# smpurkis/PyTorch-Face-Detection-from-Scratch

Hardware: AMD Instinct MI355X
Metric: train imgs/sec (PoolResnet 480^2, bs=256 per GPU) (higher is better)
Workload: dtype f32 (3x3 convs: bf16x3 split MFMA, fp32 accumulate)

## Files before the change

### pytorch-face-detection-from-scratch_amd/csrc/fdet_conv3x3_ps.hip

```cpp
#include "fdet_conv3x3_x3.h"
#include "fdet_ps.h"
#include "fdet_ldsdma.h"
#include <algorithm>

using namespace fdet;

typedef __attribute__((address_space(3))) void* lds_void_t;
typedef const __attribute__((address_space(1))) void* glb_void_t;
typedef unsigned u32x4 __attribute__((ext_vector_type(4)));

namespace {

#ifndef PS_DBG
#define PS_DBG 0
#endif
constexpr int PSA = 9 * 2 * 64;
constexpr int PS_ROWI = 10;

enum { PSE_FWD_FULL = 0, PSE_DGRAD_ACT = 1, PSE_FWD_POOL = 2, PSE_DGRAD_ADDPOOL = 3 };

struct PsConvArgs {
  const bf16x8* x;
  const bf16x8* a_hi;
  const bf16x8* a_lo;
// ... 5 lines not shown
  float* pool_f32;
  unsigned char* route_out;
  const float* dout;
  const unsigned char* route_in;
  float* dx_f32;
  int Hp, Wp, HPp, WPp, plane_p, img_p;
  int Nimg, last0, Wlast, Wf, Wpf, xo;
  unsigned magic_nimg;
  int N, H, W, HP;
  int nch, ntiles;
  int plane_i, img_i, plane_o, img_o;
  unsigned magic_hp;
  float slope;
};

typedef unsigned u32x2_t __attribute__((ext_vector_type(2)));

__device__ __forceinline__ void ps_keep(const f32x16& v) {
#if defined(__HIP_DEVICE_COMPILE__)
  asm volatile("" ::"v"(v));
#endif
}

__device__ __forceinline__ void ps_acc_read(const f32x16& acc, const int r, float& z) {
#if defined(__HIP_DEVICE_COMPILE__)
  asm("v_accvgpr_read_b32 %0, %1" : "=v"(z) : "a"(acc[r]));
#else
  z = acc[r];
#endif
}

template <int MODE, bool P16>
__device__ __forceinline__ void ps_unit(const f32x16& acc, const int gp, const float (&bza)[4], const float (&bzb)[4],
                                        const u32x2_t (&sg)[2], const float slope, const bool ok, const int ob, const int m,
                                        const int half, const int gstride, const int plane_o_bytes,
                                        const __amdgpu_buffer_rsrc_t yrs) {
  float za[4], zb[4];
#pragma unroll
  for (int i = 0; i < 4; ++i) {
#if defined(__HIP_DEVICE_COMPILE__)
    asm("v_accvgpr_read_b32 %0, %1" : "=v"(za[i]) : "a"(acc[8 * gp + i]));
    asm("v_accvgpr_read_b32 %0, %1" : "=v"(zb[i]) : "a"(acc[8 * gp + 4 + i]));
#else
    za[i] = acc[8 * gp + i]; zb[i] = acc[8 * gp + 4 + i];
#endif
  }
// ... 14 lines not shown
  unsigned ha[2], la[2], hb[2], lb[2];
  if (P16) {
    ps_hi4(za, ha);
    ps_hi4(zb, hb);
  } else {
    ps_split4(za, ha, la);
    ps_split4(zb, hb, lb);
  }
#pragma unroll
  for (int k = 0; k < 2; ++k) {
    auto r1 = __builtin_amdgcn_permlane32_swap(ha[k], hb[k], false, false);
    ha[k] = r1[0]; hb[k] = r1[1];
    if (!P16) {
      auto r2 = __builtin_amdgcn_permlane32_swap(la[k], lb[k], false, false);
      la[k] = r2[0]; lb[k] = r2[1];
    }
  }
  const int G = 4 * m + 2 * gp + half;
  const unsigned off = ok ? (unsigned)(ob + G * gstride) * 16u : 0x80000000u;
  __builtin_amdgcn_raw_buffer_store_b128(u32x4{ha[0], ha[1], hb[0], hb[1]}, yrs, off, 0, 0);
  if (!P16) __builtin_amdgcn_raw_buffer_store_b128(u32x4{la[0], la[1], lb[0], lb[1]}, yrs, off, plane_o_bytes, 0);
}

template <int MODE, int WP, bool P16>
__global__ void __launch_bounds__(256, 1)
k_conv3x3_ps(const PsConvArgs p) {
  constexpr bool WOVEN = MODE == PSE_FWD_FULL || MODE == PSE_DGRAD_ACT || MODE == PSE_DGRAD_ADDPOOL;
  extern __shared__ __attribute__((aligned(16))) char smem[];
  bf16x8* const lds = reinterpret_cast<bf16x8*>(smem);
  const int tid = threadIdx.x, lane = tid & 63;
  const int wid = __builtin_amdgcn_readfirstlane(tid >> 6);
  const int l31 = lane & 31, half = lane >> 5;
  constexpr int WPL = WP == 64 ? 6 : 5, R = 512 / WP, PT = (R + 2) * WP + 8, NBI = (R + 2) * WP / 64;
  constexpr int buf_units = 2 * PSA + 4 * PT;
  const int HP = p.HP;
  int qn[4];
#pragma unroll
  for (int n = 0; n < 4; ++n) qn[n] = WP == 64 ? (2 * wid + (n & 1)) * 64 + (n >> 1) * 32 : (4 * wid + n) * 32;
  constexpr bool POOLM = MODE == PSE_FWD_POOL || MODE == PSE_DGRAD_ADDPOOL;
  if (POOLM) {
#pragma unroll
    for (int n = 0; n < 4; ++n) qn[n] = (WP == 64 ? (2 * wid + (n >> 1)) * 64 : (4 * wid + (n >> 1)) * 32) + (n & 1);
  }
  const int lb = POOLM ? (WP == 64 ? 2 * l31 : 2 * l31 + 32 * (l31 >> 4)) : l31;
  int tile = blockIdx.x, tend = p.ntiles, tstep = gridDim.x;
  if ((gridDim.x & 7) == 0) {
    const int grp = blockIdx.x & 7, chunk = (p.ntiles + 7) >> 3;
    tile = grp * chunk + (blockIdx.x >> 3);
    tend = min((grp + 1) * chunk, p.ntiles);
// ... 24 lines not shown
    _Pragma("unroll") for (int k_ = 0; k_ < ((PS_DBG & 16) ? 0 : 9); ++k_)                          \
      dma_piece(ad_ + k_ * 1024, wvoff, wrs, (unsigned)(C) * (PSA * 16) + k_ * 1024);              \
    const unsigned bso_ = (unsigned)((wid >> 1) * p.plane_i + (2 * (C) + (wid & 1)) * HP * WP) * 16u; \
    const unsigned bd_ = db_ + (unsigned)(2 * PSA + wid * PT) * 16u;                               \
    _Pragma("unroll") for (int i_ = 0; i_ < NBI; ++i_) dma_piece(bd_ + i_ * 1024, ro[i_], xrs, bso_); \
  }

  f32x16 accA[2][4], accB[WOVEN ? 2 : 1][WOVEN ? 4 : 1];
  if (WOVEN) {
#pragma unroll
    for (int m = 0; m < 2; ++m)
#pragma unroll
      for (int n = 0; n < 4; ++n)
#pragma unroll
        for (int r = 0; r < 16; ++r) accB[WOVEN ? m : 0][WOVEN ? n : 0][r] = 0.f;
  }

  float bz[2][4][4];
#pragma unroll
  for (int m = 0; m < 2; ++m)
#pragma unroll
    for (int g = 0; g < 4; ++g)
#pragma unroll
      for (int i = 0; i < 4; ++i) bz[m][g][i] = (MODE == PSE_FWD_FULL || MODE == PSE_FWD_POOL) ? p.bias[32 * m + 8 * g + 4 * half + i] : 0.f;

  const int a_off = half * 64 + l31;
  const int b_off = 2 * PSA + half * PT + lb;
  const int gstride = HP * WP, plane_o_bytes = p.plane_o * 16;
  const __amdgpu_buffer_rsrc_t yrs = __builtin_amdgcn_make_buffer_rsrc(p.y, 0, (int)((size_t)p.N * p.img_o * 16), 0x00020000);

  int ob[4];
  bool okn[4];
#pragma unroll
  for (int n = 0; n < 4; ++n) { ob[n] = 0; okn[n] = false; }
#define PS_GEO(T)                                                                                  \
  {                                                                                                \
    _Pragma("unroll") for (int n_ = 0; n_ < 4; ++n_) {                                             \
      const int q_ = qn[n_] + l31;                                                                 \
      const int col_ = q_ & (WP - 1);                                                              \
      const int v_ = (T) * R + (q_ >> WPL);                                                        \
      const int nn_ = (int)__umulhi((unsigned)v_, p.magic_hp), y_ = v_ - nn_ * HP;                 \
      okn[n_] = nn_ < p.N && y_ < p.H && col_ < (nn_ >= p.last0 ? p.Wlast : p.W);                  \
      ob[n_] = nn_ * p.img_o + y_ * WP + col_ + 1;                                                 \
    }                                                                                              \
  }
  u32x2_t sgp[4][2][2][2];
#pragma unroll
// ... 16 lines not shown
  }

  int young = 0;
  int sb = 0;
#define PS_WAITN(K) else if (young == K) asm volatile("s_waitcnt vmcnt(" #K ")" ::: "memory");
#define PS_OPEN()                                                                                  \
  {                                                                                                \
    if (young == 0) asm volatile("s_waitcnt vmcnt(0)" ::: "memory");                               \
    PS_WAITN(4) PS_WAITN(8) PS_WAITN(12) PS_WAITN(16) PS_WAITN(32) PS_WAITN(36) PS_WAITN(40) PS_WAITN(44) PS_WAITN(48) PS_WAITN(63) \
    else asm volatile("s_waitcnt vmcnt(0)" ::: "memory");                                          \
    __builtin_amdgcn_s_barrier();                                                                  \
  }
#define PS_NEXT(C)                                                                                 \
  {                                                                                                \
    if ((C) + 1 < p.nch) {                                                                         \
      PS_DMA((C) + 1, sb ^ 1)                                                                      \
    } else if (tile + tstep < tend) {                                                              \
      PS_ROWOFF(tile + tstep)                                                                      \
      PS_DMA(0, sb ^ 1)                                                                            \
    }                                                                                              \
    __builtin_amdgcn_sched_barrier(0);                                                             \
  }
  bf16x8 ah[2][2], al[2][2], bh[2][4], bl[2][4];
#define PS_FRAGS(F, T)                                                                             \
  {                                                                                                \
    const int to_ = ((T) / 3) * WP + (T) % 3;                                                      \
    _Pragma("unroll") for (int m_ = 0; m_ < 2; ++m_) {                                             \
      ah[F][m_] = Aw[(T) * 128 + m_ * 32];                                                         \
      if (!P16) al[F][m_] = Aw[PSA + (T) * 128 + m_ * 32];                                         \
    }                                                                                              \
    _Pragma("unroll") for (int n_ = 0; n_ < 4; ++n_) {                                             \
      bh[F][n_] = Bw[qn[n_] + to_];                                                                \
      if (!P16) bl[F][n_] = Bw[2 * PT + qn[n_] + to_];                                             \
    }                                                                                              \
  }
#define PS_BODY(ACC, FIRST, JOB, PREV)                                                             \
  {                                                                                                \
    const bf16x8* buf_ = lds + sb * buf_units;                                                     \
    const bf16x8* Aw = buf_ + a_off;                                                               \
    const bf16x8* Bw = buf_ + b_off;                                                               \
    PS_FRAGS(0, 0)                                                                                 \
    __builtin_amdgcn_sched_barrier(0);                                                             \
    _Pragma("unroll") for (int t = 0; t < 9; ++t) {                                                \
      const int F = t & 1;                                                                         \
      if (t < 8) PS_FRAGS(F ^ 1, t + 1)                                                            \
      if (!(PS_DBG & 2)) {                                                                         \
        _Pragma("unroll") for (int m = 0; m < 2; ++m)                                              \
// ... 41 lines not shown
          if (i < 6) __builtin_amdgcn_sched_group_barrier(0x100, 1, 0);                            \
          if ((JOB) != 0) __builtin_amdgcn_sched_group_barrier(0x002, 6, 0);                       \
          if ((JOB) != 0 && (i >= 7 || (MODE == PSE_DGRAD_ADDPOOL && i >= 4))) __builtin_amdgcn_sched_group_barrier(0x040, 1, 0); \
        }                                                                                          \
      } else {                                                                                     \
      _Pragma("unroll") for (int i = 0; i < 12; ++i) {                                             \
        __builtin_amdgcn_sched_group_barrier(0x008, 1, 0);                                         \
        __builtin_amdgcn_sched_group_barrier(0x100, 1, 0);                                         \
        if ((JOB) != 0) __builtin_amdgcn_sched_group_barrier(0x002, 3, 0);                         \
      }                                                                                            \
      _Pragma("unroll") for (int i = 0; i < 12; ++i) {                                             \
        __builtin_amdgcn_sched_group_barrier(0x008, 1, 0);                                         \
        if ((JOB) != 0) __builtin_amdgcn_sched_group_barrier(0x002, 3, 0);                         \
        if ((JOB) != 0 && (i >= 10 || (MODE == PSE_DGRAD_ADDPOOL && i >= 8))) __builtin_amdgcn_sched_group_barrier(0x040, 1, 0); \
      }                                                                                            \
      }                                                                                            \
    }                                                                                              \
    sb ^= 1;                                                                                       \
  }
  const __amdgpu_buffer_rsrc_t prs = __builtin_amdgcn_make_buffer_rsrc(MODE == PSE_FWD_POOL ? (void*)p.pool_ps : (void*)p.dx_f32, 0,
      MODE == PSE_FWD_POOL ? (int)((size_t)p.N * p.img_p * 16) : (int)((size_t)p.Nimg * 64 * p.H * p.Wf * 4), 0x00020000);
  const __amdgpu_buffer_rsrc_t frs = __builtin_amdgcn_make_buffer_rsrc(p.pool_f32, 0, (int)((size_t)p.Nimg * 64 * p.Hp * p.Wpf * 4), 0x00020000);
  const __amdgpu_buffer_rsrc_t rrs = __builtin_amdgcn_make_buffer_rsrc(p.route_out, 0, (int)((size_t)p.N * 64 * p.Hp * p.Wp), 0x00020000);
  const int pool_cnt = MODE == PSE_FWD_POOL ? 4 * ((P16 ? 1 : 2) * (p.pool_ps != nullptr) + (p.route_out != nullptr) + 8 * (p.pool_f32 != nullptr)) : 63;
#define PS_WIN(T)                                                                                  \
    const int rb_ = WP == 64 ? 2 * wid : 4 * wid + 2 * (l31 >> 4);                                 \
    const int v_ = (T) * R + rb_;                                                                  \
    const int nn = (int)__umulhi((unsigned)v_, p.magic_hp), y = v_ - nn * HP;                      \
    const int xp = WP == 64 ? l31 : (l31 & 15), yp = y >> 1;                                       \
    const bool okw = nn < p.N && y < p.H && 2 * xp < (nn >= p.last0 ? p.Wlast : p.W);              \
                \
    const int si = p.last0 == 0 ? 0 : (p.Nimg == 1 ? nn : (int)__umulhi((unsigned)nn, p.magic_nimg)); \
    const int ni = nn - si * p.Nimg, xg = si * (p.xo >> 1) + xp;
  float dgp[2][2][2][4];
  unsigned rkp[2][2][2];
  unsigned sto = 0x80000000u;
#pragma unroll
  for (int m = 0; m < 2; ++m)
#pragma unroll
    for (int gp = 0; gp < 2; ++gp)
#pragma unroll
      for (int ab = 0; ab < 2; ++ab) {
        rkp[m][gp][ab] = 0u;
#pragma unroll
        for (int i = 0; i < 4; ++i) dgp[m][gp][ab][i] = 0.f;
      }
#define PS_POOLPREF(T)                                                                             \
  {                                                                                                \
    PS_WIN(T)                                                                                      \
    const int HWp = p.Hp * p.Wpf, HWr = p.Hp * p.Wp;                                               \
    const int pbase = okw ? (ni * 64 * p.Hp + yp) * p.Wpf + xg : 0;                                \
    const int rbase = okw ? (nn * 8 * p.Hp + yp) * p.Wp + xp : 0;                                  \
    _Pragma("unroll") for (int m = 0; m < 2; ++m)                                                  \
      _Pragma("unroll") for (int gp = 0; gp < 2; ++gp)                                             \
        _Pragma("unroll") for (int ab = 0; ab < 2; ++ab) {                                         \
          const int G = 4 * m + 2 * gp + ab;                                                       \
          _Pragma("unroll") for (int i = 0; i < 4; ++i) {                                          \
            const float v_ = p.dout[pbase + (8 * G + 4 * half + i) * HWp];                         \
            dgp[m][gp][ab][i] = okw ? v_ : 0.f;                                                    \
          }                                                                                        \
          rkp[m][gp][ab] = *reinterpret_cast<const unsigned*>(p.route_in + (size_t)(rbase + G * HWr) * 8 + 4 * half); \
        }                                                                                          \
    sto = okw ? (unsigned)(((ni * 64 + 4 * half) * p.H + y) * p.Wf + 2 * xg) * 4u : 0x80000000u;   \
  }
#define PS_EPI_FWD_POOL(ACC, T)                                                                    \
  if (!(PS_DBG & 1)) {                                                                             \
    PS_WIN(T)                                                                                      \
    const int sb0 = okw ? nn * p.img_i + y * WP + 2 * xp + 1 : 0;                                  \
    u32x2_t sk[2][2][4][4];                                                                        \
    float scv[2][2][2][4];                                                                         \
    _Pragma("unroll") for (int m = 0; m < 2; ++m)                                                  \
      _Pragma("unroll") for (int gp = 0; gp < 2; ++gp) {                                           \
        const size_t ga = (size_t)(4 * m + 2 * gp) * gstride, gb = ga + (size_t)gstride;           \
        _Pragma("unroll") for (int n = 0; n < 4; ++n) {                                            \
          const u32x2_t* ap = reinterpret_cast<const u32x2_t*>(p.aux + sb0 + (n >> 1) * WP + (n & 1)) + half; \
          sk[m][gp][n][0] = ap[ga * 2];                                                            \
          sk[m][gp][n][1] = P16 ? u32x2_t{0u, 0u} : ap[(ga + p.plane_i) * 2];                      \
          sk[m][gp][n][2] = ap[gb * 2];                                                            \
          sk[m][gp][n][3] = P16 ? u32x2_t{0u, 0u} : ap[(gb + p.plane_i) * 2];                      \
        }                                                                                          \
        _Pragma("unroll") for (int i = 0; i < 4; ++i) {                                            \
          const int ch = 32 * m + 16 * gp + 4 * half + i;                                          \
          scv[m][gp][0][i] = (p.scale && okw) ? p.scale[ni * 64 + ch] : 1.f;                       \
          scv[m][gp][1][i] = (p.scale && okw) ? p.scale[ni * 64 + ch + 8] : 1.f;                   \
        }                                                                                          \
      }                                                                                            \
     \
     \
    float pvs[2][2][2][4];                                                                         \
    unsigned rts[2][2][2];                                                                         \
    _Pragma("unroll") for (int m = 0; m < 2; ++m)                                                  \
      _Pragma("unroll") for (int gp = 0; gp < 2; ++gp) {                                           \
        unsigned rt[2] = {0u, 0u};                                                                 \
        _Pragma("unroll") for (int ab = 0; ab < 2; ++ab)                                           \
          _Pragma("unroll") for (int i = 0; i < 4; ++i) {                                          \
            float mx = -INFINITY;                                                                  \
            int arg = 0;                                                                           \
            unsigned bits = 0;                                                                     \
            _Pragma("unroll") for (int n = 0; n < 4; ++n) {                                        \
              float z;                                                                             \
              ps_acc_read(ACC[m][n], 8 * gp + 4 * ab + i, z);                                      \
              const float w_ = z + bz[m][2 * gp + ab][i];                                          \
              z = fmaxf(w_, w_ * p.slope);                                                         \
              bits |= (z > 0.f ? 1u : 0u) << n;                                                    \
              const float u_ = z * scv[m][gp][ab][i] + ps_join(sk[m][gp][n][2 * ab][i >> 1], sk[m][gp][n][2 * ab + 1][i >> 1], i & 1); \
              if (u_ > mx || u_ != u_) { mx = u_; arg = n; }    \
            }                                                                                      \
            pvs[m][gp][ab][i] = mx;                                                                \
            rt[ab] |= (bits | ((unsigned)arg << 4)) << (8 * i);                                    \
          }                                                                                        \
        rts[m][gp][0] = rt[0]; rts[m][gp][1] = rt[1];                                              \
      }                                                                                            \
    if (p.pool_f32) {                 \
      _Pragma("unroll") for (int m = 0; m < 2; ++m)                                                \
        _Pragma("unroll") for (int gp = 0; gp < 2; ++gp) {                                         \
          const unsigned off = okw ? (unsigned)(((ni * 64 + 32 * m + 16 * gp + 4 * half) * p.Hp + yp) * p.Wpf + xg) * 4u : 0x80000000u; \
          _Pragma("unroll") for (int jj = 0; jj < 8; ++jj)                                         \
            __builtin_amdgcn_raw_buffer_store_b32(__builtin_bit_cast(unsigned, pvs[m][gp][jj >> 2][jj & 3]), frs, off, \
                                                  (8 * (jj >> 2) + (jj & 3)) * p.Hp * p.Wpf * 4, 0); \
        }                                                                                          \
    }                                                                                              \
     \
    _Pragma("unroll") for (int m = 0; m < 2; ++m)                                                  \
      _Pragma("unroll") for (int gp = 0; gp < 2; ++gp) {                                           \
        _Pragma("unroll") for (int i = 0; i < 4; ++i) {                                            \
          auto r_ = __builtin_amdgcn_permlane32_swap(__float_as_uint(pvs[m][gp][0][i]), __float_as_uint(pvs[m][gp][1][i]), false, false); \
          const unsigned r0_ = r_[0], r1_ = r_[1];    \
          pvs[m][gp][0][i] = __uint_as_float(r0_); pvs[m][gp][1][i] = __uint_as_float(r1_);        \
        }                                                                                          \
        { auto r_ = __builtin_amdgcn_permlane32_swap(rts[m][gp][0], rts[m][gp][1], false, false); rts[m][gp][0] = r_[0]; rts[m][gp][1] = r_[1]; } \
      }                                                                                            \
    if (p.pool_ps) {                                                                               \
      _Pragma("unroll") for (int m = 0; m < 2; ++m)                                                \
        _Pragma("unroll") for (int gp = 0; gp < 2; ++gp) {                                         \
          const int G = 4 * m + 2 * gp + half;                                                     \
          unsigned ha[2], la[2], hb[2], lb2[2];                                                    \
          if (P16) { ps_hi4(pvs[m][gp][0], ha); ps_hi4(pvs[m][gp][1], hb); }                       \
          else { ps_split4(pvs[m][gp][0], ha, la); ps_split4(pvs[m][gp][1], hb, lb2); }            \
          const unsigned off = okw ? (unsigned)(nn * p.img_p + (G * p.HPp + yp) * p.WPp + xp + 1) * 16u : 0x80000000u; \
          __builtin_amdgcn_raw_buffer_store_b128(u32x4{ha[0], ha[1], hb[0], hb[1]}, prs, off, 0, 0); \
          if (!P16) __builtin_amdgcn_raw_buffer_store_b128(u32x4{la[0], la[1], lb2[0], lb2[1]}, prs, off, p.plane_p * 16, 0); \
        }                                                                                          \
    }                                                                                              \
    if (p.route_out) {                                                                             \
      _Pragma("unroll") for (int m = 0; m < 2; ++m)                                                \
        _Pragma("unroll") for (int gp = 0; gp < 2; ++gp) {                                         \
          const int G = 4 * m + 2 * gp + half;                                                     \
          const unsigned off = okw ? (unsigned)(((nn * 8 + G) * p.Hp + yp) * p.Wp + xp) * 8u : 0x80000000u; \
          __builtin_amdgcn_raw_buffer_store_b64(u32x2_t{rts[m][gp][0], rts[m][gp][1]}, rrs, off, 0, 0); \
        }                                                                                          \
    }                                                                                              \
  } else {                                                                                         \
    _Pragma("unroll") for (int m = 0; m < 2; ++m)                                                  \
      _Pragma("unroll") for (int n = 0; n < 4; ++n) ps_keep(ACC[m][n]);                            \
  }
#define PS_EPI_ADDPOOL(ACC, T)                                                                     \
  if (!(PS_DBG & 1)) {                                                                             \
    PS_WIN(T)                                                                                      \
    float dg[2][2][2][4];                                                                          \
    unsigned rk[2][2][2];                                                                          \
    const int HWp = p.Hp * p.Wpf;                                                                  \
    const int pbase = okw ? (ni * 64 * p.Hp + yp) * p.Wpf + xg : 0;                                \
    _Pragma("unroll") for (int m = 0; m < 2; ++m)                                                  \
      _Pragma("unroll") for (int gp = 0; gp < 2; ++gp)                                             \
        _Pragma("unroll") for (int ab = 0; ab < 2; ++ab) {                                         \
          const int G = 4 * m + 2 * gp + ab;                                                       \
          _Pragma("unroll") for (int i = 0; i < 4; ++i) dg[m][gp][ab][i] = okw ? p.dout[pbase + (8 * G + 4 * half + i) * HWp] : 0.f; \
          rk[m][gp][ab] = okw ? *reinterpret_cast<const unsigned*>(p.route_in + (size_t)(((nn * 8 + G) * p.Hp + yp) * p.Wp + xp) * 8 + 4 * half) : 0u; \
        }                                                                                          \
    _Pragma("unroll") for (int m = 0; m < 2; ++m)                                                  \
      _Pragma("unroll") for (int gp = 0; gp < 2; ++gp)                                             \
        _Pragma("unroll") for (int ab = 0; ab < 2; ++ab)                                           \
          _Pragma("unroll") for (int i = 0; i < 4; ++i) {                                          \
// ... 41 lines not shown
      PS_OPEN()                                                                                    \
      PS_NEXT(c)                                                                                   \
      PS_BODY(ACC, 0, 0, PREV)                                                                     \
      young = 0;                                                                                   \
    }                                                                                              \
    PS_GEO(tile)                                                                                   \
    etile = tile;                                                                                  \
    if (WOVEN && MODE == PSE_DGRAD_ACT && !(PS_DBG & 1)) {                                         \
      PS_SIGNS()                                                                                   \
      young += 32;                                                                                 \
    }                                                                                              \
    if constexpr (MODE == PSE_DGRAD_ADDPOOL) {                                                     \
      if (!(PS_DBG & 1)) {                                                                         \
        PS_POOLPREF(tile)                                                                          \
        young = min(young + 40, 63);                                                               \
      }                                                                                            \
    }                                                                                              \
    if (!WOVEN) {                                                                                  \
      PS_EPILOGUE(ACC)                                                                             \
      young = (PS_DBG & 1) ? 0 : (POOLM ? pool_cnt : 32);                                          \
    }                                                                                              \
  }

  int etile = tile;
  PS_ROWOFF(tile)
  PS_DMA(0, 0)
  if (WOVEN) {
    for (;;) {
      PS_TILE(accA, accB)
      tile += tstep;
      if (tile >= tend) { PS_EPILOGUE(accA) break; }
      PS_TILE(accB, accA)
      tile += tstep;
      if (tile >= tend) { PS_EPILOGUE(accB) break; }
    }
  } else {
    for (; tile < tend; tile += tstep) PS_TILE(accA, accA)
  }
#undef PS_TILE
#undef PS_EPILOGUE
#undef PS_EPI_ADDPOOL
#undef PS_EPI_FWD_POOL
#undef PS_POOLPREF
#undef PS_WIN
#undef PS_WAITN
#undef PS_BODY
#undef PS_FRAGS
#undef PS_NEXT
#undef PS_OPEN
#undef PS_GEO
#undef PS_SIGNS
#undef PS_DMA
#undef PS_ROWOFF
}

#ifndef PS_TU
#define PS_TU (-1)
#endif
#define PS_CAT_(a, b) a##b
#define PS_CAT(a, b) PS_CAT_(a, b)
#define PS_TU_NAME PS_CAT(fdet_ps_launch_, PS_TU)
template <int MODE, int WP, bool P16>
int launch_ps(const PsConvArgs& p, size_t lds, int grid, hipStream_t st) {
  static bool attr_set = false;
  constexpr int lds_max = 2 * (2 * PSA + 4 * 648) * 16;
  if (!attr_set) {
    if ((int)lds > lds_max || hipFuncSetAttribute((const void*)k_conv3x3_ps<MODE, WP, P16>, hipFuncAttributeMaxDynamicSharedMemorySize, lds_max) != hipSuccess) {
      (void)hipGetLastError();
      return fail(FDET_ELAUNCH, "conv3x3_ps: cannot reserve %zu bytes of LDS", lds);
    }
    attr_set = true;
  }
  hipLaunchKernelGGL((k_conv3x3_ps<MODE, WP, P16>), dim3(grid), dim3(256), lds, st, p);
  return check_launch("fdet_conv3x3_ps");
}

}
#define PS_DECL_LAUNCH(N) extern "C" int fdet_ps_launch_##N(const void* args, size_t lds, int grid, void* stream);
PS_DECL_LAUNCH(0) PS_DECL_LAUNCH(1) PS_DECL_LAUNCH(2) PS_DECL_LAUNCH(3) PS_DECL_LAUNCH(4) PS_DECL_LAUNCH(5) PS_DECL_LAUNCH(6) PS_DECL_LAUNCH(7)
PS_DECL_LAUNCH(8) PS_DECL_LAUNCH(9) PS_DECL_LAUNCH(10) PS_DECL_LAUNCH(11) PS_DECL_LAUNCH(12) PS_DECL_LAUNCH(13) PS_DECL_LAUNCH(14) PS_DECL_LAUNCH(15)
#if PS_TU >= 0
extern "C" int PS_TU_NAME(const void* args, size_t lds, int grid, void* stream) {
  return launch_ps<(PS_TU & 7) / 2, (PS_TU & 1) ? 64 : 32, (PS_TU >= 8)>(*reinterpret_cast<const PsConvArgs*>(args), lds, grid, (hipStream_t)stream);
}
#endif
namespace {
#if PS_TU == -1
typedef int (*ps_launch_fn)(const void*, size_t, int, void*);
const ps_launch_fn PS_LAUNCHERS[16] = {fdet_ps_launch_0, fdet_ps_launch_1, fdet_ps_launch_2, fdet_ps_launch_3,
                                       fdet_ps_launch_4, fdet_ps_launch_5, fdet_ps_launch_6, fdet_ps_launch_7,
                                       fdet_ps_launch_8, fdet_ps_launch_9, fdet_ps_launch_10, fdet_ps_launch_11,
                                       fdet_ps_launch_12, fdet_ps_launch_13, fdet_ps_launch_14, fdet_ps_launch_15};
struct PsPoolIO {
  const float* scale = nullptr; void* pool_ps = nullptr; float* pool_f32 = nullptr; unsigned char* route_out = nullptr;
  const float* dout = nullptr; const unsigned char* route_in = nullptr; float* dx_f32 = nullptr;
};

const char* ps_conv_refusal(int pooled, int N, int Cin, int Cout, int H, int W) {
  PsGeo gi, go, gp;
  PsStrips sp, spo;
  if (!(Cout == 64 && Cin % 16 == 0 && Cin >= 32)) return "Cout must be 64 and Cin a multiple of 16, at least 32";
  if (!(ps_geo_strips(N, Cin, H, W, gi, sp) && ps_geo_strips(N, Cout, H, W, go, spo) && gi.WP >= 32 && sp.Ws + 2 <= gi.WP))
    return "unsupported map (W + 2 <= 32 or 64 slots, or an even width in strips)";
  if (!((size_t)(gi.N + 2) * gi.img * 16 < ((size_t)1 << 32) && (size_t)(go.N + 2) * go.img * 16 < ((size_t)1 << 32)))
    return "tensor too large for the 32-bit byte offsets of the DMA descriptors";
  if (pooled) {
    if ((H & 1) || (W & 1) || Cin != 64) return "pooled block: even map and 64 channels required";
    if ((size_t)N * 64 * H * W * 4 >= ((size_t)1 << 31)) return "pooled block: tensor too large for 32-bit offsets";
    if (pooled == 2 && sp.S != 1) return "a strip map writes its pooled output as fp32 NCHW (pool_f32)";
    if (pooled == 2 && !ps_geo(gi.N, 64, H / 2, W / 2, gp)) return "the pooled map has no PS layout";
  }
  if ((long)gi.N * gi.HP + gi.HP >= (1 << 20)) return "too many rows";
  return nullptr;
}

// ... 18 lines not shown
  p.bias = bias;
  p.y = reinterpret_cast<bf16x8*>(y);
  p.aux = reinterpret_cast<const bf16x8*>(aux);
  p.scale = io.scale; p.pool_ps = reinterpret_cast<bf16x8*>(io.pool_ps); p.pool_f32 = io.pool_f32; p.route_out = io.route_out;
  p.dout = io.dout; p.route_in = io.route_in; p.dx_f32 = io.dx_f32;
  p.Hp = H / 2; p.Wp = W / 2; p.HPp = p.WPp = p.plane_p = p.img_p = 0;
  p.Nimg = Nimg; p.last0 = sp.S > 1 ? (sp.S - 1) * Nimg : 0; p.Wlast = sp.Wlast; p.Wf = Wfull; p.Wpf = Wfull / 2; p.xo = sp.Ws;
  p.magic_nimg = Nimg > 1 ? magic_of(Nimg) : 0u;
  PsGeo go;
  PsStrips spo;
  ps_geo_strips(Nimg, Cout, H, Wfull, go, spo);
  if (pool_mode == 2) {
    ps_geo(N, 64, H / 2, W / 2, gp);
    p.HPp = gp.HP; p.WPp = gp.WP; p.plane_p = gp.plane; p.img_p = gp.img;
  }
  p.N = N; p.H = H; p.W = W; p.HP = gi.HP;
  p.nch = Cin / 16;
  const int R = 512 / gi.WP, PT = (R + 2) * gi.WP + 8;
  const long vr = (long)N * gi.HP;
  p.ntiles = (int)((vr + R - 1) / R);
  p.plane_i = gi.plane; p.img_i = gi.img; p.plane_o = go.plane; p.img_o = go.img;
  p.magic_hp = magic_of(gi.HP);
  p.slope = slope;
  const size_t lds = (size_t)2 * (2 * PSA + 4 * PT) * 16;
  const int grid = std::min(p.ntiles, num_cus());
  const bool w64 = gi.WP == 64;
  switch (mode) {
    case PSE_FWD_FULL:
      FDET_REQUIRE(bias, "conv3x3_ps_fwd: bias is required");
      break;
    case PSE_DGRAD_ACT:
      FDET_REQUIRE(aux, "conv3x3_ps_dgrad_act: the activation is required");
      break;
    case PSE_FWD_POOL:
      FDET_REQUIRE(bias && aux && (io.pool_ps || io.pool_f32), "conv3x3_ps_fwd_pool: bias, skip and an output are required");
      break;
    default:
      FDET_REQUIRE(io.dout && io.route_in && io.dx_f32, "conv3x3_ps_dgrad_unpool: dout, route and dx are required");
      break;
  }
  return PS_LAUNCHERS[(p16 ? 8 : 0) + 2 * mode + (w64 ? 1 : 0)](&p, lds, grid, (void*)st);
}
#endif

}

#if PS_TU == -1
extern "C" int fdet_conv3x3_ps_ok(int N, int Cin, int Cout, int H, int W, int pooled) {
  return ps_conv_refusal(pooled, N, Cin, Cout, H, W) == nullptr;
}

extern "C" int fdet_conv3x3_ps_fwd(const void* x_ps, const void* wpk, const float* bias, void* y_ps, int N, int Cin,
                                   int Cout, int H, int W, float slope, void* stream) {
  return run_ps(PSE_FWD_FULL, x_ps, wpk, bias, nullptr, y_ps, PsPoolIO{}, N, Cin, Cout, H, W, slope, (hipStream_t)stream);
}

extern "C" int fdet_conv3x3_ps_dgrad_act(const void* dz_ps, const void* wpk, const void* act_ps, void* dx_ps, int N,
                                         int Cin, int Cout, int H, int W, float slope, void* stream) {
  return run_ps(PSE_DGRAD_ACT, dz_ps, wpk, nullptr, act_ps, dx_ps, PsPoolIO{}, N, Cout, Cin, H, W, slope, (hipStream_t)stream);
}

extern "C" int fdet_conv3x3_ps_fwd_pool(const void* x_ps, const void* wpk, const float* bias, const void* skip_ps,
                                        const float* drop_scale, void* pool_ps, float* pool_f32, unsigned char* route8,
// ... 39 lines not shown
```

Baseline: 94280.

## Run pooled forward conv with two workgroups per CU using single-buffered LDS

Result: faster. 95940 (median of 6 runs) (+1.8%).

```diff
diff --git a/pytorch-face-detection-from-scratch_amd/csrc/fdet_conv3x3_ps.hip b/pytorch-face-detection-from-scratch_amd/csrc/fdet_conv3x3_ps.hip
--- a/pytorch-face-detection-from-scratch_amd/csrc/fdet_conv3x3_ps.hip
+++ b/pytorch-face-detection-from-scratch_amd/csrc/fdet_conv3x3_ps.hip
@@ -51,6 +51,20 @@
 #endif
 }
 
+__device__ __forceinline__ void ps_opaque(unsigned& v) {
+#if defined(__HIP_DEVICE_COMPILE__)
+  asm("" : "+v"(v));
+#endif
+}
+
+__device__ __forceinline__ int ps_lane_now() {
+  int v = 0;
+#if defined(__HIP_DEVICE_COMPILE__)
+  asm volatile("v_mbcnt_lo_u32_b32 %0, -1, 0\n\tv_mbcnt_hi_u32_b32 %0, -1, %0" : "=v"(v));
+#endif
+  return v;
+}
+
 __device__ __forceinline__ void ps_acc_read(const f32x16& acc, const int r, float& z) {
 #if defined(__HIP_DEVICE_COMPILE__)
   asm("v_accvgpr_read_b32 %0, %1" : "=v"(z) : "a"(acc[r]));
@@ -111,9 +125,10 @@
   if (!P16) __builtin_amdgcn_raw_buffer_store_b128(u32x4{la[0], la[1], lb[0], lb[1]}, yrs, off, plane_o_bytes, 0);
 }
 
-template <int MODE, int WP, bool P16>
-__global__ void __launch_bounds__(256, 1)
+template <int MODE, int WP, bool P16, bool WG2 = false>
+__global__ void __launch_bounds__(256, WG2 ? 2 : 1)
 k_conv3x3_ps(const PsConvArgs p) {
+  static_assert(!WG2 || MODE == PSE_FWD_POOL, "two workgroups per CU: the pooled forward only (one accumulator set)");
   constexpr bool WOVEN = MODE == PSE_FWD_FULL || MODE == PSE_DGRAD_ACT || MODE == PSE_DGRAD_ADDPOOL;
   extern __shared__ __attribute__((aligned(16))) char smem[];
   bf16x8* const lds = reinterpret_cast<bf16x8*>(smem);
@@ -184,7 +199,7 @@
 #pragma unroll
     for (int g = 0; g < 4; ++g)
 #pragma unroll
-      for (int i = 0; i < 4; ++i) bz[m][g][i] = (MODE == PSE_FWD_FULL || MODE == PSE_FWD_POOL) ? p.bias[32 * m + 8 * g + 4 * half + i] : 0.f;
+      for (int i = 0; i < 4; ++i) bz[m][g][i] = ((MODE == PSE_FWD_FULL || MODE == PSE_FWD_POOL) && !WG2) ? p.bias[32 * m + 8 * g + 4 * half + i] : 0.f;
 
   const int a_off = half * 64 + l31;
   const int b_off = 2 * PSA + half * PT + lb;
@@ -247,7 +262,47 @@
     __builtin_amdgcn_sched_barrier(0);                                                             \
   }
   bf16x8 ah[2][2], al[2][2], bh[2][4], bl[2][4];
-#define PS_FRAGS(F, T)                                                                             \
+#define PS_FRAG_A(F, T)                                                                            \
+  {                                                                                                \
+    _Pragma("unroll") for (int m_ = 0; m_ < 2; ++m_) {                                             \
+      ah[F][m_] = Aw[(T) * 128 + m_ * 32];                                                         \
+      if (!P16) al[F][m_] = Aw[PSA + (T) * 128 + m_ * 32];                                         \
+    }                                                                                              \
+  }
+#define PS_FRAG_B(N, T)                                                                            \
+  {                                                                                                \
+    const int to_ = ((T) / 3) * WP + (T) % 3;                                                      \
+    bh[0][N] = Bw[qn[N] + to_];                                                                    \
+    if (!P16) bl[0][N] = Bw[2 * PT + qn[N] + to_];                                                 \
+  }
+#define PS_BODY2(ACC, FIRST)                                                                       \
+  {                                                                                                \
+    const bf16x8* Aw = lds + a_off;                                                                \
+    const bf16x8* Bw = lds + b_off;                                                                \
+    PS_FRAG_A(0, 0)                                                                                \
+    _Pragma("unroll") for (int n = 0; n < 4; ++n) PS_FRAG_B(n, 0)                                  \
+    __builtin_amdgcn_sched_barrier(0);                                                             \
+    _Pragma("unroll") for (int t = 0; t < 9; ++t) {                                                \
+      const int F = t & 1;                                                                         \
+      if (t < 8) PS_FRAG_A(F ^ 1, t + 1)                                                           \
+      _Pragma("unroll") for (int n = 0; n < 4; ++n) {                                              \
+        if (!(PS_DBG & 2)) {                                                                       \
+          _Pragma("unroll") for (int m = 0; m < 2; ++m) {                                          \
+            const f32x16 zero_ = {};                                                               \
+            if (P16) {                                                                             \
+              ACC[m][n] = __builtin_amdgcn_mfma_f32_32x32x16_bf16(ah[F][m], bh[0][n], ((FIRST) && t == 0) ? zero_ : ACC[m][n], 0, 0, 0); \
+            } else {                                                                               \
+              ACC[m][n] = __builtin_amdgcn_mfma_f32_32x32x16_bf16(ah[F][m], bl[0][n], ((FIRST) && t == 0) ? zero_ : ACC[m][n], 0, 0, 0); \
+              ACC[m][n] = __builtin_amdgcn_mfma_f32_32x32x16_bf16(al[F][m], bh[0][n], ACC[m][n], 0, 0, 0); \
+              ACC[m][n] = __builtin_amdgcn_mfma_f32_32x32x16_bf16(ah[F][m], bh[0][n], ACC[m][n], 0, 0, 0); \
+            }                                                                                      \
+          }                                                                                        \
+        }                                                                                          \
+        if (t < 8) PS_FRAG_B(n, t + 1)                                                             \
+      }                                                                                            \
+    }                                                                                              \
+  }
+#define PS_FRAGS(F, T)                                                                         \
   {                                                                                                \
     const int to_ = ((T) / 3) * WP + (T) % 3;                                                      \
     _Pragma("unroll") for (int m_ = 0; m_ < 2; ++m_) {                                             \
@@ -335,6 +390,9 @@
       MODE == PSE_FWD_POOL ? (int)((size_t)p.N * p.img_p * 16) : (int)((size_t)p.Nimg * 64 * p.H * p.Wf * 4), 0x00020000);
   const __amdgpu_buffer_rsrc_t frs = __builtin_amdgcn_make_buffer_rsrc(p.pool_f32, 0, (int)((size_t)p.Nimg * 64 * p.Hp * p.Wpf * 4), 0x00020000);
   const __amdgpu_buffer_rsrc_t rrs = __builtin_amdgcn_make_buffer_rsrc(p.route_out, 0, (int)((size_t)p.N * 64 * p.Hp * p.Wp), 0x00020000);
+  const __amdgpu_buffer_rsrc_t srs = __builtin_amdgcn_make_buffer_rsrc((void*)p.scale, 0, (WG2 && p.scale) ? (int)((size_t)p.Nimg * 64 * 4) : 0, 0x00020000);
+  const __amdgpu_buffer_rsrc_t ars = __builtin_amdgcn_make_buffer_rsrc((void*)p.aux, 0, WG2 ? (int)((size_t)p.N * p.img_i * 16) : 0, 0x00020000);
+  const __amdgpu_buffer_rsrc_t brs = __builtin_amdgcn_make_buffer_rsrc((void*)p.bias, 0, (WG2 && p.bias) ? 64 * 4 : 0, 0x00020000);
   const int pool_cnt = MODE == PSE_FWD_POOL ? 4 * ((P16 ? 1 : 2) * (p.pool_ps != nullptr) + (p.route_out != nullptr) + 8 * (p.pool_f32 != nullptr)) : 63;
 #define PS_WIN(T)                                                                                  \
     const int rb_ = WP == 64 ? 2 * wid : 4 * wid + 2 * (l31 >> 4);                                 \
@@ -376,28 +434,97 @@
         }                                                                                          \
     sto = okw ? (unsigned)(((ni * 64 + 4 * half) * p.H + y) * p.Wf + 2 * xg) * 4u : 0x80000000u;   \
   }
+#define PS_EPI_LOADS(M, GP)                                                                        \
+  {                                                                                                \
+    const size_t ga = (size_t)(4 * (M) + 2 * (GP)) * gstride, gb = ga + (size_t)gstride;           \
+    _Pragma("unroll") for (int n = 0; n < 4; ++n) {                                                \
+      const u32x2_t* ap = reinterpret_cast<const u32x2_t*>(p.aux + sb0 + (n >> 1) * WP + (n & 1)) + half; \
+      sk[M][GP][n][0] = ap[ga * 2];                                                                \
+      sk[M][GP][n][1] = P16 ? u32x2_t{0u, 0u} : ap[(ga + p.plane_i) * 2];                          \
+      sk[M][GP][n][2] = ap[gb * 2];                                                                \
+      sk[M][GP][n][3] = P16 ? u32x2_t{0u, 0u} : ap[(gb + p.plane_i) * 2];                          \
+    }                                                                                              \
+    _Pragma("unroll") for (int i = 0; i < 4; ++i) {                                                \
+      const int ch = 32 * (M) + 16 * (GP) + 4 * half + i;                                          \
+      scv[M][GP][0][i] = (p.scale && okw) ? p.scale[ni * 64 + ch] : 1.f;                           \
+      scv[M][GP][1][i] = (p.scale && okw) ? p.scale[ni * 64 + ch + 8] : 1.f;                       \
+      bzw[M][2 * (GP)][i] = bz[M][2 * (GP)][i];                                                    \
+      bzw[M][2 * (GP) + 1][i] = bz[M][2 * (GP) + 1][i];                                            \
+    }                                                                                              \
+  }
+#define PS_EPI_LOADS_G(M, GP, AB)                                                                  \
+  {                                                                                                \
+    const int g_ = (4 * (M) + 2 * (GP) + (AB)) * gstride * 16;                                     \
+    _Pragma("unroll") for (int n = 0; n < 4; ++n) {    \
+      const int n_ = ((n >> 1) * WP + (n & 1)) * 16;                                               \
+      sk[M][GP][n][2 * (AB)] = __builtin_amdgcn_raw_buffer_load_b64(ars, skoff, g_ + n_, 0);       \
+      sk[M][GP][n][2 * (AB) + 1] = P16 ? u32x2_t{0u, 0u} : __builtin_amdgcn_raw_buffer_load_b64(ars, skoff, g_ + p.plane_i * 16 + n_, 0); \
+    }                                                                                              \
+    _Pragma("unroll") for (int i = 0; i < 4; ++i) {                                                \
+      const int ch = 32 * (M) + 16 * (GP) + 8 * (AB) + i;                                          \
+      const unsigned sv_ = __builtin_amdgcn_raw_buffer_load_b32(srs, scoff, ch * 4, 0);            \
+      scv[M][GP][AB][i] = __uint_as_float((sv_ & scm) | (0x3f800000u & ~scm));    \
+      bzw[M][2 * (GP) + (AB)][i] = __uint_as_float(__builtin_amdgcn_raw_buffer_load_b32(brs, (unsigned)halfe * 16u, ch * 4, 0)); \
+    }                                                                                              \
+  }
+#define PS_EPI_ST_F32(M, GP)                                                                       \
+  {                                                                                                \
+    const unsigned off = okw ? (unsigned)(((ni * 64 + 32 * (M) + 16 * (GP) + 4 * halfe) * p.Hp + yp) * p.Wpf + xg) * 4u : 0x80000000u;\
+    _Pragma("unroll") for (int jj = 0; jj < 8; ++jj)                                               \
+      __builtin_amdgcn_raw_buffer_store_b32(__builtin_bit_cast(unsigned, pvs[M][GP][jj >> 2][jj & 3]), frs, off,\
+                                            (8 * (jj >> 2) + (jj & 3)) * p.Hp * p.Wpf * 4, 0);     \
+  }
+#define PS_EPI_XCHG(M, GP)                                                                         \
+  {                                                                                                \
+    _Pragma("unroll") for (int i = 0; i < 4; ++i) {                                                \
+      auto r_ = __builtin_amdgcn_permlane32_swap(__float_as_uint(pvs[M][GP][0][i]), __float_as_uint(pvs[M][GP][1][i]), false, false);\
+      const unsigned r0_ = r_[0], r1_ = r_[1];   \
+      pvs[M][GP][0][i] = __uint_as_float(r0_); pvs[M][GP][1][i] = __uint_as_float(r1_);            \
+    }                                                                                              \
+    { auto r_ = __builtin_amdgcn_permlane32_swap(rts[M][GP][0], rts[M][GP][1], false, false); rts[M][GP][0] = r_[0]; rts[M][GP][1] = r_[1]; }\
+  }
+#define PS_EPI_ST_PS(M, GP)                                                                        \
+  {                                                                                                \
+    const int G = 4 * (M) + 2 * (GP) + halfe;                                                       \
+    unsigned ha[2], la[2], hb[2], lb2[2];                                                          \
+    if (P16) { ps_hi4(pvs[M][GP][0], ha); ps_hi4(pvs[M][GP][1], hb); }                             \
+    else { ps_split4(pvs[M][GP][0], ha, la); ps_split4(pvs[M][GP][1], hb, lb2); }                  \
+    const unsigned off = okw ? (unsigned)(nn * p.img_p + (G * p.HPp + yp) * p.WPp + xp + 1) * 16u : 0x80000000u;\
+    __builtin_amdgcn_raw_buffer_store_b128(u32x4{ha[0], ha[1], hb[0], hb[1]}, prs, off, 0, 0);     \
+    if (!P16) __builtin_amdgcn_raw_buffer_store_b128(u32x4{la[0], la[1], lb2[0], lb2[1]}, prs, off, p.plane_p * 16, 0);\
+  }
+#define PS_EPI_ST_RT(M, GP)                                                                        \
+  {                                                                                                \
+    const int G = 4 * (M) + 2 * (GP) + halfe;                                                       \
+    const unsigned off = okw ? (unsigned)(((nn * 8 + G) * p.Hp + yp) * p.Wp + xp) * 8u : 0x80000000u;\
+    __builtin_amdgcn_raw_buffer_store_b64(u32x2_t{rts[M][GP][0], rts[M][GP][1]}, rrs, off, 0, 0);  \
+  }
 #define PS_EPI_FWD_POOL(ACC, T)                                                                    \
   if (!(PS_DBG & 1)) {                                                                             \
+    \
+    \
+    const int l31o_ = l31, halfo_ = half;                                                          \
+    {                                                                                              \
+    int l31 = l31o_, halfe = halfo_;                                                               \
+    if (WG2) {                                                                                     \
+      const int ln_ = ps_lane_now();                                                               \
+      l31 = ln_ & 31; halfe = ln_ >> 5;                                                            \
+    }                                                                                              \
     PS_WIN(T)                                                                                      \
     const int sb0 = okw ? nn * p.img_i + y * WP + 2 * xp + 1 : 0;                                  \
     u32x2_t sk[2][2][4][4];                                                                        \
-    float scv[2][2][2][4];                                                                         \
-    _Pragma("unroll") for (int m = 0; m < 2; ++m)                                                  \
-      _Pragma("unroll") for (int gp = 0; gp < 2; ++gp) {                                           \
-        const size_t ga = (size_t)(4 * m + 2 * gp) * gstride, gb = ga + (size_t)gstride;           \
-        _Pragma("unroll") for (int n = 0; n < 4; ++n) {                                            \
-          const u32x2_t* ap = reinterpret_cast<const u32x2_t*>(p.aux + sb0 + (n >> 1) * WP + (n & 1)) + half; \
-          sk[m][gp][n][0] = ap[ga * 2];                                                            \
-          sk[m][gp][n][1] = P16 ? u32x2_t{0u, 0u} : ap[(ga + p.plane_i) * 2];                      \
-          sk[m][gp][n][2] = ap[gb * 2];                                                            \
-          sk[m][gp][n][3] = P16 ? u32x2_t{0u, 0u} : ap[(gb + p.plane_i) * 2];                      \
-        }                                                                                          \
-        _Pragma("unroll") for (int i = 0; i < 4; ++i) {                                            \
-          const int ch = 32 * m + 16 * gp + 4 * half + i;                                          \
-          scv[m][gp][0][i] = (p.scale && okw) ? p.scale[ni * 64 + ch] : 1.f;                       \
-          scv[m][gp][1][i] = (p.scale && okw) ? p.scale[ni * 64 + ch + 8] : 1.f;                   \
-        }                                                                                          \
-      }                                                                                            \
+    float scv[2][2][2][4], bzw[2][4][4];                                                           \
+    const unsigned scoff = okw ? (unsigned)(ni * 64 + 4 * halfe) * 4u : 0x80000000u;                \
+    const unsigned skoff = (unsigned)sb0 * 16u + (unsigned)halfe * 8u;                              \
+    unsigned scm = (p.scale && okw) ? 0xffffffffu : 0u;                                            \
+    ps_opaque(scm);    \
+                       \
+    if (!WG2) {                         \
+      _Pragma("unroll") for (int m = 0; m < 2; ++m)                                                \
+        _Pragma("unroll") for (int gp = 0; gp < 2; ++gp) PS_EPI_LOADS(m, gp)                       \
+    } else {             \
+      PS_EPI_LOADS_G(0, 0, 0)                                                                      \
+    }                                                                                              \
      \
      \
     float pvs[2][2][2][4];                                                                         \
@@ -405,7 +532,12 @@
     _Pragma("unroll") for (int m = 0; m < 2; ++m)                                                  \
       _Pragma("unroll") for (int gp = 0; gp < 2; ++gp) {                                           \
         unsigned rt[2] = {0u, 0u};                                                                 \
-        _Pragma("unroll") for (int ab = 0; ab < 2; ++ab)                                           \
+        _Pragma("unroll") for (int ab = 0; ab < 2; ++ab) {                                         \
+          if (WG2) {                                                                               \
+            const int s1_ = 4 * m + 2 * gp + ab + 1;                                               \
+            __builtin_amdgcn_sched_barrier(0);                                                     \
+            if (s1_ < 8) PS_EPI_LOADS_G((s1_ >> 2) & 1, (s1_ >> 1) & 1, s1_ & 1)                   \
+          }                                                                                        \
           _Pragma("unroll") for (int i = 0; i < 4; ++i) {                                          \
             float mx = -INFINITY;                                                                  \
             int arg = 0;                                                                           \
@@ -413,7 +545,7 @@
             _Pragma("unroll") for (int n = 0; n < 4; ++n) {                                        \
               float z;                                                                             \
               ps_acc_read(ACC[m][n], 8 * gp + 4 * ab + i, z);                                      \
-              const float w_ = z + bz[m][2 * gp + ab][i];                                          \
+              const float w_ = z + bzw[m][2 * gp + ab][i];                                         \
               z = fmaxf(w_, w_ * p.slope);                                                         \
               bits |= (z > 0.f ? 1u : 0u) << n;                                                    \
               const float u_ = z * scv[m][gp][ab][i] + ps_join(sk[m][gp][n][2 * ab][i >> 1], sk[m][gp][n][2 * ab + 1][i >> 1], i & 1); \
@@ -421,47 +553,33 @@
             }                                                                                      \
             pvs[m][gp][ab][i] = mx;                                                                \
             rt[ab] |= (bits | ((unsigned)arg << 4)) << (8 * i);                                    \
+            if (WG2) __builtin_amdgcn_sched_barrier(0);    \
           }                                                                                        \
+        }                                                                                          \
         rts[m][gp][0] = rt[0]; rts[m][gp][1] = rt[1];                                              \
-      }                                                                                            \
-    if (p.pool_f32) {                 \
+        if (WG2) {   \
+          if (p.pool_f32) PS_EPI_ST_F32(m, gp)                                                     \
+          PS_EPI_XCHG(m, gp)                                                                       \
+          if (p.pool_ps) PS_EPI_ST_PS(m, gp)                                                       \
+          if (p.route_out) PS_EPI_ST_RT(m, gp)                                                     \
+        }                                                                                          \
+      }                                                                                            \
+    if (!WG2) {                                                                                    \
+      if (p.pool_f32) {                                                                            \
+        _Pragma("unroll") for (int m = 0; m < 2; ++m)                                              \
+          _Pragma("unroll") for (int gp = 0; gp < 2; ++gp) PS_EPI_ST_F32(m, gp)                    \
+      }                                                                                            \
       _Pragma("unroll") for (int m = 0; m < 2; ++m)                                                \
-        _Pragma("unroll") for (int gp = 0; gp < 2; ++gp) {                                         \
-          const unsigned off = okw ? (unsigned)(((ni * 64 + 32 * m + 16 * gp + 4 * half) * p.Hp + yp) * p.Wpf + xg) * 4u : 0x80000000u; \
-          _Pragma("unroll") for (int jj = 0; jj < 8; ++jj)                                         \
-            __builtin_amdgcn_raw_buffer_store_b32(__builtin_bit_cast(unsigned, pvs[m][gp][jj >> 2][jj & 3]), frs, off, \
-                                                  (8 * (jj >> 2) + (jj & 3)) * p.Hp * p.Wpf * 4, 0); \
-        }                                                                                          \
-    }                                                                                              \
-     \
-    _Pragma("unroll") for (int m = 0; m < 2; ++m)                                                  \
-      _Pragma("unroll") for (int gp = 0; gp < 2; ++gp) {                                           \
-        _Pragma("unroll") for (int i = 0; i < 4; ++i) {                                            \
-          auto r_ = __builtin_amdgcn_permlane32_swap(__float_as_uint(pvs[m][gp][0][i]), __float_as_uint(pvs[m][gp][1][i]), false, false); \
-          const unsigned r0_ = r_[0], r1_ = r_[1];    \
-          pvs[m][gp][0][i] = __uint_as_float(r0_); pvs[m][gp][1][i] = __uint_as_float(r1_);        \
-        }                                                                                          \
-        { auto r_ = __builtin_amdgcn_permlane32_swap(rts[m][gp][0], rts[m][gp][1], false, false); rts[m][gp][0] = r_[0]; rts[m][gp][1] = r_[1]; } \
-      }                                                                                            \
-    if (p.pool_ps) {                                                                               \
-      _Pragma("unroll") for (int m = 0; m < 2; ++m)                                                \
-        _Pragma("unroll") for (int gp = 0; gp < 2; ++gp) {                                         \
-          const int G = 4 * m + 2 * gp + half;                                                     \
-          unsigned ha[2], la[2], hb[2], lb2[2];                                                    \
-          if (P16) { ps_hi4(pvs[m][gp][0], ha); ps_hi4(pvs[m][gp][1], hb); }                       \
-          else { ps_split4(pvs[m][gp][0], ha, la); ps_split4(pvs[m][gp][1], hb, lb2); }            \
-          const unsigned off = okw ? (unsigned)(nn * p.img_p + (G * p.HPp + yp) * p.WPp + xp + 1) * 16u : 0x80000000u; \
-          __builtin_amdgcn_raw_buffer_store_b128(u32x4{ha[0], ha[1], hb[0], hb[1]}, prs, off, 0, 0); \
-          if (!P16) __builtin_amdgcn_raw_buffer_store_b128(u32x4{la[0], la[1], lb2[0], lb2[1]}, prs, off, p.plane_p * 16, 0); \
-        }                                                                                          \
-    }                                                                                              \
-    if (p.route_out) {                                                                             \
-      _Pragma("unroll") for (int m = 0; m < 2; ++m)                                                \
-        _Pragma("unroll") for (int gp = 0; gp < 2; ++gp) {                                         \
-          const int G = 4 * m + 2 * gp + half;                                                     \
-          const unsigned off = okw ? (unsigned)(((nn * 8 + G) * p.Hp + yp) * p.Wp + xp) * 8u : 0x80000000u; \
-          __builtin_amdgcn_raw_buffer_store_b64(u32x2_t{rts[m][gp][0], rts[m][gp][1]}, rrs, off, 0, 0); \
-        }                                                                                          \
+        _Pragma("unroll") for (int gp = 0; gp < 2; ++gp) PS_EPI_XCHG(m, gp)                        \
+      if (p.pool_ps) {                                                                             \
+        _Pragma("unroll") for (int m = 0; m < 2; ++m)                                              \
+          _Pragma("unroll") for (int gp = 0; gp < 2; ++gp) PS_EPI_ST_PS(m, gp)                     \
+      }                                                                                            \
+      if (p.route_out) {                                                                           \
+        _Pragma("unroll") for (int m = 0; m < 2; ++m)                                              \
+          _Pragma("unroll") for (int gp = 0; gp < 2; ++gp) PS_EPI_ST_RT(m, gp)                     \
+      }                                                                                            \
+    }                                                                                              \
     }                                                                                              \
   } else {                                                                                         \
     _Pragma("unroll") for (int m = 0; m < 2; ++m)                                                  \
@@ -549,10 +667,36 @@
     }                                                                                              \
   }
 
+#define PS_TILE2(ACC)                                                                              \
+  {                                                                                                \
+    PS_OPEN()                                                                                      \
+    PS_BODY2(ACC, 1)                                                                               \
+    for (int c = 1; c < p.nch; ++c) {                                                              \
+      __builtin_amdgcn_s_barrier();                                                                \
+      { const int lane = ps_lane_now(); PS_ROWOFF(tile) }   \
+      PS_DMA(c, 0)                                                                                 \
+      __builtin_amdgcn_sched_barrier(0);                                                           \
+      asm volatile("s_waitcnt vmcnt(0)" ::: "memory");                                             \
+      __builtin_amdgcn_s_barrier();                                                                \
+      PS_BODY2(ACC, 0)                                                                             \
+    }                                                                                              \
+    __builtin_amdgcn_s_barrier();                                                                  \
+    if (tile + tstep < tend) {                                                                     \
+      { const int lane = ps_lane_now(); PS_ROWOFF(tile + tstep) }                                  \
+      PS_DMA(0, 0)                                                                                 \
+    }                                                                                              \
+    __builtin_amdgcn_sched_barrier(0);                                                             \
+    etile = tile;                                                                                  \
+    PS_EPILOGUE(ACC)                                                                               \
+    young = (PS_DBG & 1) ? 0 : pool_cnt;                                                           \
+  }
+
   int etile = tile;
   PS_ROWOFF(tile)
   PS_DMA(0, 0)
-  if (WOVEN) {
+  if constexpr (WG2) {
+    for (; tile < tend; tile += tstep) PS_TILE2(accA)
+  } else if (WOVEN) {
     for (;;) {
       PS_TILE(accA, accB)
       tile += tstep;
@@ -564,10 +708,20 @@
   } else {
     for (; tile < tend; tile += tstep) PS_TILE(accA, accA)
   }
+#undef PS_TILE2
 #undef PS_TILE
 #undef PS_EPILOGUE
 #undef PS_EPI_ADDPOOL
 #undef PS_EPI_FWD_POOL
+#undef PS_EPI_ST_RT
+#undef PS_EPI_ST_PS
+#undef PS_EPI_XCHG
+#undef PS_EPI_ST_F32
+#undef PS_EPI_LOADS_G
+#undef PS_EPI_LOADS
+#undef PS_BODY2
+#undef PS_FRAG_B
+#undef PS_FRAG_A
 #undef PS_POOLPREF
 #undef PS_WIN
 #undef PS_WAITN
@@ -587,18 +741,18 @@
 #define PS_CAT_(a, b) a##b
 #define PS_CAT(a, b) PS_CAT_(a, b)
 #define PS_TU_NAME PS_CAT(fdet_ps_launch_, PS_TU)
-template <int MODE, int WP, bool P16>
+template <int MODE, int WP, bool P16, bool WG2 = false>
 int launch_ps(const PsConvArgs& p, size_t lds, int grid, hipStream_t st) {
   static bool attr_set = false;
-  constexpr int lds_max = 2 * (2 * PSA + 4 * 648) * 16;
+  constexpr int lds_max = (WG2 ? 1 : 2) * (2 * PSA + 4 * 648) * 16;
   if (!attr_set) {
-    if ((int)lds > lds_max || hipFuncSetAttribute((const void*)k_conv3x3_ps<MODE, WP, P16>, hipFuncAttributeMaxDynamicSharedMemorySize, lds_max) != hipSuccess) {
+    if ((int)lds > lds_max || hipFuncSetAttribute((const void*)k_conv3x3_ps<MODE, WP, P16, WG2>, hipFuncAttributeMaxDynamicSharedMemorySize, lds_max) != hipSuccess) {
       (void)hipGetLastError();
       return fail(FDET_ELAUNCH, "conv3x3_ps: cannot reserve %zu bytes of LDS", lds);
     }
     attr_set = true;
   }
-  hipLaunchKernelGGL((k_conv3x3_ps<MODE, WP, P16>), dim3(grid), dim3(256), lds, st, p);
+  hipLaunchKernelGGL((k_conv3x3_ps<MODE, WP, P16, WG2>), dim3(grid), dim3(256), lds, st, p);
   return check_launch("fdet_conv3x3_ps");
 }
 
@@ -606,9 +760,15 @@
 #define PS_DECL_LAUNCH(N) extern "C" int fdet_ps_launch_##N(const void* args, size_t lds, int grid, void* stream);
 PS_DECL_LAUNCH(0) PS_DECL_LAUNCH(1) PS_DECL_LAUNCH(2) PS_DECL_LAUNCH(3) PS_DECL_LAUNCH(4) PS_DECL_LAUNCH(5) PS_DECL_LAUNCH(6) PS_DECL_LAUNCH(7)
 PS_DECL_LAUNCH(8) PS_DECL_LAUNCH(9) PS_DECL_LAUNCH(10) PS_DECL_LAUNCH(11) PS_DECL_LAUNCH(12) PS_DECL_LAUNCH(13) PS_DECL_LAUNCH(14) PS_DECL_LAUNCH(15)
+PS_DECL_LAUNCH(wg2_4) PS_DECL_LAUNCH(wg2_5)
 #if PS_TU >= 0
 extern "C" int PS_TU_NAME(const void* args, size_t lds, int grid, void* stream) {
   return launch_ps<(PS_TU & 7) / 2, (PS_TU & 1) ? 64 : 32, (PS_TU >= 8)>(*reinterpret_cast<const PsConvArgs*>(args), lds, grid, (hipStream_t)stream);
+}
+#endif
+#if PS_TU == 4 || PS_TU == 5
+extern "C" int PS_CAT(fdet_ps_launch_wg2_, PS_TU)(const void* args, size_t lds, int grid, void* stream) {
+  return launch_ps<PSE_FWD_POOL, (PS_TU & 1) ? 64 : 32, false, true>(*reinterpret_cast<const PsConvArgs*>(args), lds, grid, (hipStream_t)stream);
 }
 #endif
 namespace {
@@ -618,6 +778,7 @@
                                        fdet_ps_launch_4, fdet_ps_launch_5, fdet_ps_launch_6, fdet_ps_launch_7,
                                        fdet_ps_launch_8, fdet_ps_launch_9, fdet_ps_launch_10, fdet_ps_launch_11,
                                        fdet_ps_launch_12, fdet_ps_launch_13, fdet_ps_launch_14, fdet_ps_launch_15};
+constexpr bool PS_WG2_DEFAULT_64 = true, PS_WG2_DEFAULT_32 = true;
 struct PsPoolIO {
   const float* scale = nullptr; void* pool_ps = nullptr; float* pool_f32 = nullptr; unsigned char* route_out = nullptr;
   const float* dout = nullptr; const unsigned char* route_in = nullptr; float* dx_f32 = nullptr;
@@ -682,9 +843,16 @@
   p.plane_i = gi.plane; p.img_i = gi.img; p.plane_o = go.plane; p.img_o = go.img;
   p.magic_hp = magic_of(gi.HP);
   p.slope = slope;
-  const size_t lds = (size_t)2 * (2 * PSA + 4 * PT) * 16;
-  const int grid = std::min(p.ntiles, num_cus());
+  size_t lds = (size_t)2 * (2 * PSA + 4 * PT) * 16;
+  int grid = std::min(p.ntiles, num_cus());
   const bool w64 = gi.WP == 64;
+  static const int wg2_env = [] { const char* e = getenv("FDET_PS_POOL_WG2"); return (e && (e[0] == '0' || e[0] == '1') && !e[1]) ? e[0] - '0' : -1; }();
+  bool wg2 = mode == PSE_FWD_POOL && !p16 && (wg2_env >= 0 ? wg2_env == 1 : (w64 ? PS_WG2_DEFAULT_64 : PS_WG2_DEFAULT_32));
+  if (wg2 && 2 * (lds / 2) > (size_t)160 * 1024) wg2 = false;
+  if (wg2) {
+    lds /= 2;
+    grid = std::min(p.ntiles, 2 * num_cus());
+  }
   switch (mode) {
     case PSE_FWD_FULL:
       FDET_REQUIRE(bias, "conv3x3_ps_fwd: bias is required");
@@ -699,6 +867,7 @@
       FDET_REQUIRE(io.dout && io.route_in && io.dx_f32, "conv3x3_ps_dgrad_unpool: dout, route and dx are required");
       break;
   }
+  if (wg2) return (w64 ? fdet_ps_launch_wg2_5 : fdet_ps_launch_wg2_4)(&p, lds, grid, (void*)st);
   return PS_LAUNCHERS[(p16 ? 8 : 0) + 2 * mode + (w64 ? 1 : 0)](&p, lds, grid, (void*)st);
 }
 #endif
```
